# kasirershahartau/tissue_image_processing

Measured on AMD Instinct MI355X. Metric: frames/sec end-to-end (2048^2, z=30), higher is better.
Workload: dtype f32(f16x3)

## Files before the change

include/tissue_hip.h:

```cpp
#ifndef TISSUE_HIP_H
#define TISSUE_HIP_H

#include <stddef.h>
#include <stdint.h>

#ifdef __cplusplus
extern "C" {
#endif

#define TIP_API __attribute__((visibility("default")))

typedef enum {
    TIP_OK = 0,
    TIP_ERR_HIP = -1,
    TIP_ERR_ARG = -2,
    TIP_ERR_NOMEM = -3,
    TIP_ERR_INDEX = -4,
    TIP_ERR_UNSUPPORTED = -5,
    TIP_ERR_OVERFLOW = -6
} tip_status;

TIP_API int tip_init(int device);
TIP_API int tip_shutdown(void);
TIP_API int tip_last_error(char *buf, size_t n);
// ... 52 lines not shown
                                     int ref_ch, int airyscan, int atoh_shift,
                                     const double *t05, const double *t1, const double *t2, const double *t30,
                                     const unsigned long long *hist_dev, double *proj, int64_t *zmap);

TIP_API int tip_bias_relu_affine_f32_dev(float *x, const float *bias, const float *scale, const float *shift, long n, int c,
                                         void *stream);
TIP_API int tip_pointer_device(const void *p);
TIP_API int tip_wait_stream(void *stream);
TIP_API int tip_stream_wait_tip(void *stream);
typedef struct tip_unet_conv_desc {
    const void *in0, *in1;
    int c0, c1, h, w, planes;
    const void *weights;
    int ntaps, dy[9], dx[9];
    int cout;
    const float *bias, *scale, *shift;
    void *out;
    int out_h, out_w, sy, sx, oy, ox;
    void *pool_out;
    const float *head_w, *head_b;
    float *head_out;
    int format;
    float acc_scale;
} tip_unet_conv_desc;
TIP_API int tip_unet_conv_dev(const tip_unet_conv_desc *d, void *stream);
TIP_API int tip_unet_conv_first_dev(const float *in, int h, int w, const float *wgt, const float *bias, const float *scale,
                                    const float *shift, void *out, int planes, int format, void *stream);
TIP_API int tip_unet_pool2_dev(const void *in, int h, int w, int ch, int planes, int format, void *out, void *stream);
TIP_API int tip_unet_head_dev(const void *in, long npix, const float *wgt, const float *bias, float *out, int planes, int format,
                              int logits, void *stream);
TIP_API int tip_unet_prepare_f64_dev(const double *img, int c, int a, int b, long cstride, long sa, long sb, int kind, float *out,
                                     int ap, int bp, void *stream);
TIP_API int tip_unet_tail_dev(const void *p, int dtype, long ld, int y, int x, double thr, int32_t *labels, double *hc,
                              int32_t *flags_host);

TIP_API int tip_draw_cell_types_u8(const uint8_t *types, long n, int must_mask, int lack_mask, const double *pos_rgb,
                                   const double *neg_rgb, double *out3);
TIP_API int tip_draw_tracking_i32(const int32_t *track, long n, const double *cycle18, double *out3);
TIP_API int tip_draw_disks_f64(int y, int x, int n, const double *cy, const double *cx, double radius, const double *rgb, double *out3);
TIP_API int tip_draw_lines_f64(int y, int x, int n, const int32_t *ends, const double *rgb, double *out3);

TIP_API int tip_rankfilter2d(const void *in, void *out, int dtype , int y, int x, int ky, int kx,
                             int footprint_kind, int border_mode, int is_max);
TIP_API int tip_rankfilter2d_dev(const void *in, void *out, int dtype, int y, int x, int ky, int kx,
                                 int footprint_kind, int border_mode, int is_max);
TIP_API int tip_local_threshold_f64_dev(const double *img, double *out, int y, int x, double imgthresh, int block);

TIP_API int tip_label4_i32(const int32_t *in, int32_t bg, int32_t *out, int y, int x, int32_t *n_labels);
// ... 58 lines not shown
```

tissue_image_processing_amd/_unet_hip.py:

```python
import ctypes
import os
import threading

import numpy as np

from . import _lib

_MODES = {
    "f16x3": (2, 1, 3, "7.2e-7"),
    "bf16x3": (2, 0, 3, "1.6e-5"),
    "bf16x6": (3, 0, 6, "9e-8"),
}
_F16_ACT_SCALE = 16.0


class _ConvDesc(ctypes.Structure):
    _fields_ = [("in0", ctypes.c_void_p), ("in1", ctypes.c_void_p), ("c0", ctypes.c_int), ("c1", ctypes.c_int), ("h", ctypes.c_int),
                ("w", ctypes.c_int), ("planes", ctypes.c_int), ("weights", ctypes.c_void_p), ("ntaps", ctypes.c_int),
                ("dy", ctypes.c_int * 9), ("dx", ctypes.c_int * 9), ("cout", ctypes.c_int), ("bias", ctypes.c_void_p),
                ("scale", ctypes.c_void_p), ("shift", ctypes.c_void_p), ("out", ctypes.c_void_p), ("out_h", ctypes.c_int),
                ("out_w", ctypes.c_int), ("sy", ctypes.c_int), ("sx", ctypes.c_int), ("oy", ctypes.c_int), ("ox", ctypes.c_int),
                ("pool_out", ctypes.c_void_p), ("head_w", ctypes.c_void_p), ("head_b", ctypes.c_void_p), ("head_out", ctypes.c_void_p),
                ("format", ctypes.c_int), ("acc_scale", ctypes.c_float)]


def split_pack(taps, planes, fmt=0):
    import torch
    T, cin, cout = taps.shape
    pieces, rest = [], taps.float()
    for _ in range(planes):
        h = rest.to(torch.float16 if fmt else torch.bfloat16)
        pieces.append(h)
        rest = rest - h.float()
    row = torch.arange(32, device=taps.device)
    chan = 16 * ((row >> 2) & 1) + 4 * (row >> 3) + (row & 3)
    pk = torch.stack(pieces, 0).view(planes, T, cin // 16, 16, cout // 32, 32)[..., chan]
    pk = pk.reshape(planes, T, cin // 16, 16, cout // 128, 128)
    return pk.permute(1, 2, 4, 0, 5, 3).contiguous()


def weights(net, mode):
    hw = net._hipw.get(mode)
    if hw is not None:
        return hw
    torch = net.torch
    p = net.p
    planes, fmt = _MODES[mode][:2]
    act = _F16_ACT_SCALE if fmt else 1.0
    hw = {}

    def pack(taps, bias_only):
        if not fmt:
            return split_pack(taps, planes), 1.0
        big = float(taps.abs().max())
        wscale = 2.0 ** (14 - int(np.floor(np.log2(big)))) if big > 0 and np.isfinite(big) else 1.0
        inv = 1.0 / (act * wscale)
        return split_pack(taps * wscale, planes, fmt), (inv * act if bias_only else inv)

    def conv3(name):
        w = p[name + ".w"].float()
        taps = torch.stack([w[:, :, ky, kx].t() for ky in range(3) for kx in range(3)], 0)
        wp, inv = pack(taps, False)
        hw[name] = (wp, [ky - 1 for ky in range(3) for kx in range(3)], [kx - 1 for ky in range(3) for kx in range(3)], inv)

    def conv_t(name):
        w = p[name + ".w"].float()
        per_axis = {0: [(0, 0), (2, -1)], 1: [(1, 0)]}
        for py in (0, 1):
            for px in (0, 1):
                tl = [(ky, dy, kx, dx) for ky, dy in per_axis[py] for kx, dx in per_axis[px]]
                taps = torch.stack([w[:, :, ky, kx] for ky, _, kx, _ in tl], 0)
                wp, inv = pack(taps, True)
                hw["%s.%d%d" % (name, py, px)] = (wp, [t[1] for t in tl], [t[3] for t in tl], inv)

    for blk in ("d0", "d1", "d2", "mid", "u0", "u1", "u2"):
        if blk != "d0":
            conv3(blk + ".c1")
        conv3(blk + ".c2")
    for i in range(3):
        conv_t("u%d.t" % i)
    w0 = p["d0.c1.w"].float()
    hw["first"] = w0.permute(2, 3, 1, 0).reshape(18, 128).contiguous()
    hw["head"] = (p["head.w"].float().reshape(2, 128) / act).contiguous()
    for k in list(p):
        if k.endswith((".b", ".s", ".t")) and not k.endswith(".t.w"):
            v = p[k].float().reshape(-1)
            scaled = k.endswith((".s", ".t", ".t.b"))
            hw["f:" + k] = (v * act if scaled else v).contiguous()
    net._hipw[mode] = hw
    return hw


_FORWARD_GATES = {}
_FORWARD_GATES_LOCK = threading.Lock()


def _forward_gate(device_index):
    with _FORWARD_GATES_LOCK:
        g = _FORWARD_GATES.get(device_index)
        if g is None:
            g = _FORWARD_GATES[device_index] = {"lock": threading.Lock(), "event": None, "stream": None}
        return g


def forward(net, x, mode, logits):
    torch = net.torch
    if os.environ.get("TISSUE_HIP_UNET_SERIAL", "1") == "0":
        return _launch(net, x, mode, logits)
    gate = _forward_gate(x.device.index)
    with gate["lock"]:
        s = torch.cuda.current_stream(x.device)
        if gate["event"] is not None and gate["stream"] != s.cuda_stream:
            s.wait_event(gate["event"])
        out = _launch(net, x, mode, logits)
        ev = torch.cuda.Event()
        ev.record(s)
        gate["event"], gate["stream"] = ev, s.cuda_stream
    return out


def _conv_desc(layer, planes, fmt, src, skip, h, w, bias, scale=None, shift=None, out=None, out_h=None, out_w=None, stride=1, oy=0, ox=0,
               pooled=None, head=None):
    wp, dy, dx, inv = layer
    d = _ConvDesc()
    d.format, d.acc_scale = fmt, inv
    d.in0, d.c0 = src.data_ptr(), src.shape[3]
    d.in1, d.c1 = (skip.data_ptr(), skip.shape[3]) if skip is not None else (None, 0)
    d.h, d.w, d.planes = h, w, planes
    d.weights, d.ntaps, d.cout = wp.data_ptr(), len(dy), wp.shape[2] * 128
    for i in range(len(dy)):
        d.dy[i], d.dx[i] = dy[i], dx[i]
    d.bias = bias.data_ptr()
    d.scale, d.shift = (scale.data_ptr(), shift.data_ptr()) if scale is not None else (None, None)
    if head is not None:
        d.head_w, d.head_b, d.head_out = (t.data_ptr() for t in head)
    d.out = out.data_ptr() if out is not None else None
    d.out_h, d.out_w = (h, w) if out_h is None else (out_h, out_w)
    d.sy, d.sx, d.oy, d.ox = stride, stride, oy, ox
    d.pool_out = pooled.data_ptr() if pooled is not None else None
    return d


def _launch(net, x, mode, logits):
    torch = net.torch
    planes, fmt = _MODES[mode][:2]
    hw = weights(net, mode)
    net.last_mode = mode
    lib = _lib.lib()
    stream = ctypes.c_void_p(torch.cuda.current_stream(x.device).cuda_stream)
    H, W = int(x.shape[2]), int(x.shape[3])
    x = x.to(torch.float32).contiguous()
    D = lambda t: ctypes.c_void_p(t.data_ptr())
    trace = getattr(net, "trace", None)

    def timed(name, flop, fn):
        if trace is None:
            return fn()
        e0, e1 = torch.cuda.Event(enable_timing=True), torch.cuda.Event(enable_timing=True)
        e0.record()
        r = fn()
        e1.record()
        trace.append((name, flop, e0, e1))
        return r

    def buf(h, w, c):
        return torch.empty((planes, h, w, c), dtype=torch.float16 if fmt else torch.bfloat16, device=x.device)

    def launch_conv(name, d):
        timed("%s %dx%d %d+%d->%d x%d taps" % (name, d.h, d.w, d.c0, d.c1, d.cout, d.ntaps), 2.0 * d.h * d.w * d.ntaps * d.cout * (d.c0 + d.c1),
              lambda: _lib.check(lib.tip_unet_conv_dev(ctypes.byref(d), stream)))

    def conv3(name, bn, src, skip, h, w, pooled=None, head=None):
        out = buf(h, w, hw[name][0].shape[2] * 128) if head is None else None
        launch_conv(name, _conv_desc(hw[name], planes, fmt, src, skip, h, w, hw["f:" + name + ".b"], hw["f:" + bn + ".s"], hw["f:" + bn + ".t"],
                                     out=out, pooled=pooled, head=None if head is None else (hw["head"], hw["f:head.b"], head)))
        return out

    def first(h, w):
        out = buf(h, w, 128)
        timed("first %dx%d 2->128" % (h, w), 2.0 * h * w * 18 * 128,
              lambda: _lib.check(lib.tip_unet_conv_first_dev(D(x), h, w, D(hw["first"]), D(hw["f:d0.c1.b"]), D(hw["f:d0.b1.s"]),
                                                             D(hw["f:d0.b1.t"]), D(out), planes, fmt, stream)))
        return out

    def double(blk, src, skip, h, w, pooled=None, head=None):
        a = first(h, w) if src is None else conv3(blk + ".c1", blk + ".b1", src, skip, h, w)
        return conv3(blk + ".c2", blk + ".b2", a, None, h, w, pooled=pooled, head=head)

    def conv_t(name, src, h, w):
        up = buf(2 * h, 2 * w, hw[name + ".00"][0].shape[2] * 128)
        for py in (0, 1):
            for px in (0, 1):
                cls = "%s.%d%d" % (name, py, px)
                launch_conv(cls, _conv_desc(hw[cls], planes, fmt, src, None, h, w, hw["f:" + name + ".b"], out=up, out_h=2 * h, out_w=2 * w,
                                            stride=2, oy=py, ox=px))
        return up

    with torch.no_grad():
        skips, cur, h, w = [], None, H, W
        for i in range(3):
            pooled = buf(h // 2, w // 2, net.filters[i])
            skips.append(double("d%d" % i, cur, None, h, w, pooled=pooled))
            cur, h, w = pooled, h // 2, w // 2
        cur = double("mid", cur, None, h, w)
        for i in range(3):
            up = conv_t("u%d.t" % i, cur, h, w)
            h, w = 2 * h, 2 * w
            probs = None
            if i == 2 and not logits and not os.environ.get("TISSUE_HIP_UNET_SEPARATE_HEAD"):
                probs = torch.empty((1, 2, H, W), dtype=torch.float32, device=x.device)
            cur = double("u%d" % i, up, skips[2 - i], h, w, head=probs)
        if probs is not None:
            return probs
        out = torch.empty((1, 2, H, W), dtype=torch.float32, device=x.device)
        timed("head %dx%d" % (H, W), 2.0 * H * W * 256,
              lambda: _lib.check(lib.tip_unet_head_dev(D(cur), ctypes.c_long(H * W), D(hw["head"]), D(hw["f:head.b"]), D(out), planes, fmt,
                                                       1 if logits else 0, stream)))
    return out
```

tissue_image_processing_amd/csrc/tip_unet.hip:

```cpp
#include "tip_internal.h"
#include "tip_unet_conv.h"
#include <algorithm>
#include <atomic>

namespace tip {

__global__ void __launch_bounds__(256) k_bias_relu_affine_f32(float *__restrict__ x, const float *__restrict__ bias,
                                                              const float *__restrict__ scale, const float *__restrict__ shift,
                                                              long n4, int C)
{
    const long i = (long)blockIdx.x * blockDim.x + threadIdx.x;
    if (i >= n4) return;
    float4 v = reinterpret_cast<float4 *>(x)[i];
    const int c = (int)((i * 4) % C);
    const float4 b = *reinterpret_cast<const float4 *>(bias + c);
    const float4 s = *reinterpret_cast<const float4 *>(scale + c);
    const float4 t = *reinterpret_cast<const float4 *>(shift + c);
    v.x += b.x; v.y += b.y; v.z += b.z; v.w += b.w;
    v.x = v.x > 0.f ? v.x : 0.f; v.y = v.y > 0.f ? v.y : 0.f; v.z = v.z > 0.f ? v.z : 0.f; v.w = v.w > 0.f ? v.w : 0.f;
    v.x = v.x * s.x + t.x; v.y = v.y * s.y + t.y; v.z = v.z * s.z + t.z; v.w = v.w * s.w + t.w;
    reinterpret_cast<float4 *>(x)[i] = v;
}

int rankfilter2d_dev(const void *in, void *out, int dtype, int Y, int X, int ky, int kx, int fp, int border, int is_max);
// ... 341 lines not shown
    split(1.0 / 100.0, r1, g1);
    split(99.0 / 100.0, r99, g99);
    hipLaunchKernelGGL(k_prep_reset, dim3(1), dim3(64), 0, s, st, c, r1, r99);
    const dim3 hgrid((unsigned)cdiv(n, 2048), (unsigned)c);
    for (int shift = 56; shift >= 0; shift -= 8) {
        hipLaunchKernelGGL(k_prep_hist, hgrid, dim3(256), 0, s, img, cstride, n, st, shift);
        hipLaunchKernelGGL(k_prep_pick, dim3(1), dim3(64), 0, s, st, c, shift);
    }
    hipLaunchKernelGGL(k_prep_next, hgrid, dim3(256), 0, s, img, cstride, n, st);
    hipLaunchKernelGGL(k_prep_finish, dim3(1), dim3(64), 0, s, st, c, g1, g99, kind);
    if (ap != a || bp != b) TIP_HIP(hipMemsetAsync(out, 0, (size_t)c * ap * bp * sizeof(float), s));
    const dim3 ngrid((unsigned)cdiv(a, 32), (unsigned)cdiv(b, 32), (unsigned)c);
    if (a_contig)
        hipLaunchKernelGGL(k_prep_normalize<true>, ngrid, dim3(256), 0, s, img, cstride, sa, sb, a, b, (const PrepState *)st, kind == 1 ? 1 : 0, out, ap, bp, ap - a, bp - b);
    else
        hipLaunchKernelGGL(k_prep_normalize<false>, ngrid, dim3(256), 0, s, img, cstride, sa, sb, a, b, (const PrepState *)st, kind == 1 ? 1 : 0, out, ap, bp, ap - a, bp - b);
    return unet_launch_check("unet_prepare");
}

int tip_unet_conv_dev(const tip_unet_conv_desc *d, void *stream)
{
    Ctx &c = ctx();
    if (!c.stream) return TIP_ERR_HIP;
    if (!d || !d->in0 || !d->weights || !d->bias || (!d->out && !d->head_out)) return fail(TIP_ERR_ARG, "tip_unet_conv_dev: null pointer");
    if (d->planes != 2 && d->planes != 3) return fail(TIP_ERR_ARG, "tip_unet_conv_dev: planes must be 2 or 3");
    if (d->format != 0 && d->format != 1) return fail(TIP_ERR_ARG, "tip_unet_conv_dev: format is 0 (bf16 pieces) or 1 (fp16 pieces)");
    if (d->format == 1 && (d->planes != 2 || !(d->acc_scale > 0.f))) return fail(TIP_ERR_ARG, "tip_unet_conv_dev: fp16 pieces come in two planes with a positive acc_scale");
    if (d->h < 8 || d->w < UC_TW || d->h % 8 || d->w % UC_TW)
        return fail(TIP_ERR_UNSUPPORTED, "tip_unet_conv_dev: the grid %dx%d is not a multiple of the 8x%d pixel tile", d->h, d->w, UC_TW);
    if (d->c0 < UC_KC || d->c0 % UC_KC || d->c1 < 0 || d->c1 % UC_KC || (d->c1 > 0 && !d->in1) || d->cout < UC_BN || d->cout % UC_BN)
        return fail(TIP_ERR_UNSUPPORTED, "tip_unet_conv_dev: channels (%d + %d -> %d) must be multiples of %d / %d", d->c0, d->c1, d->cout, UC_KC, UC_BN);
    if (d->ntaps < 1 || d->ntaps > 9 || d->sy < 1 || d->sx < 1 || d->oy < 0 || d->ox < 0 ||
        (d->h - 1) * d->sy + d->oy >= d->out_h || (d->w - 1) * d->sx + d->ox >= d->out_w)
        return fail(TIP_ERR_ARG, "tip_unet_conv_dev: bad taps / output mapping");
    if ((d->scale == nullptr) != (d->shift == nullptr)) return fail(TIP_ERR_ARG, "tip_unet_conv_dev: scale and shift come together");
    if (18L * d->w * (d->c0 > d->c1 ? d->c0 : d->c1) * 2 >= (1L << 32) - 65536)
        return fail(TIP_ERR_UNSUPPORTED, "tip_unet_conv_dev: 18 rows of %d pixels x %d channels exceed the 4 GB a buffer resource addresses",
                    d->w, d->c0 > d->c1 ? d->c0 : d->c1);
    ConvParams p;
    p.in0 = (const uint16_t *)d->in0; p.in1 = (const uint16_t *)(d->c1 > 0 ? d->in1 : d->in0);
    p.c0 = d->c0; p.c1 = d->c1; p.H = d->h; p.W = d->w;
    p.w = (const uint16_t *)d->weights; p.ntaps = d->ntaps;
    for (int t = 0; t < 9; ++t) {
        p.dy[t] = t < d->ntaps ? d->dy[t] : 0; p.dx[t] = t < d->ntaps ? d->dx[t] : 0;
        if (p.dy[t] < -1 || p.dy[t] > 1 || p.dx[t] < -1 || p.dx[t] > 1) return fail(TIP_ERR_ARG, "tip_unet_conv_dev: tap offsets are -1, 0 or 1");
    }
    p.cout = d->cout; p.bias = d->bias; p.scale = d->scale; p.shift = d->shift;
    p.out = (uint16_t *)d->out; p.outH = d->out_h; p.outW = d->out_w; p.sy = d->sy; p.sx = d->sx; p.oy = d->oy; p.ox = d->ox;
    p.pool_out = (uint16_t *)d->pool_out;
    p.acc_scale = d->format == 1 ? d->acc_scale : 1.f;
#ifdef UC_TRACE
    static unsigned long long *trace_dev = nullptr;
    if (!trace_dev) { TIP_HIP(hipMalloc(&trace_dev, 1024)); }
    TIP_HIP(hipMemsetAsync(trace_dev, 0, 1024, (hipStream_t)stream));
    p.trace = trace_dev;
#endif
    p.head_w = d->head_w; p.head_b = d->head_b; p.head_out = d->head_out;
    if (d->head_out && (!d->head_w || !d->head_b || d->cout != UC_BN || !d->scale || d->pool_out || d->sy != 1 || d->sx != 1 || d->oy != 0 || d->ox != 0 ||
                        d->out_h != d->h || d->out_w != d->w))
        return fail(TIP_ERR_ARG, "tip_unet_conv_dev: the fused head needs a 128-channel Conv2D + BatchNorm layer with the plain output mapping");
    if (d->pool_out && (d->sy != 1 || d->sx != 1 || d->oy != 0 || d->ox != 0 || d->out_h != d->h || d->out_w != d->w))
        return fail(TIP_ERR_ARG, "tip_unet_conv_dev: pool_out needs the plain output mapping");
    const int t8 = tuning().unet_tile8;
    const bool want8 = t8 == 1 || (t8 < 0 && d->ntaps == 9 && d->c0 + d->c1 <= 128);
    const int th = (d->planes == 2 && d->h % 16 == 0 && !want8) ? 16 : 8;
    const int dist = (th == 16 && d->ntaps >= 4) ? 4 : 2;
    const int da = (th == 16 && d->ntaps <= 2) ? 2 : 1;
    const int threads = th * 32, hp = UC_HW * (th + 2);
    const int ntiles = (d->h / th) * (d->w / UC_TW), nblks = d->cout / UC_BN;
    p.xcd_map = (tuning().unet_xcd_map && nblks > 1 && ntiles % 8 == 0) ? 1 : 0;
    const dim3 grid = p.xcd_map ? dim3((unsigned)(ntiles * nblks)) : dim3(ntiles, nblks);
    const int a_per = (d->planes * ((hp * 2 + 63) / 64) * 64 + threads - 1) / threads;
    const int spb = (th == 16 && dist == 4 && d->ntaps == 9 && tuning().unet_spb > 1) ? 3 : 1;
    const size_t lds = (size_t)(da + 1) * a_per * threads * 16 + (size_t)(spb > 1 ? 3 * spb : dist + 1) * d->planes * 256 * 16;
    hipStream_t s = (hipStream_t)stream;
    int which;
    if (d->planes == 3) which = 3;
    else if (th == 8) which = 0;
    else if (spb == 3) which = 6;
    else if (dist == 4) which = 2;
    else if (da == 2) which = 4;
    else which = 1;
    static std::atomic<unsigned> attr_done[64];
    const unsigned bit = 1u << (which + (d->format ? 9 : 0));
    const int dev = c.device >= 0 && c.device < 64 ? c.device : 0;
// ... 21 lines not shown
            UC_FLAVOUR(4, k_unet_conv<2, 16, 2, 2, 1, true>)
            UC_FLAVOUR(1, k_unet_conv<2, 16, 2, 1, 1, true>)
            UC_FLAVOUR(0, k_unet_conv<2, 8, 2, 1, 1, true>)
        }
    }
#undef UC_FLAVOUR
#ifdef UC_TRACE
    {
        unsigned long long tr[128];
        TIP_HIP(hipStreamSynchronize(s));
        TIP_HIP(hipMemcpy(tr, trace_dev, sizeof tr, hipMemcpyDeviceToHost));
        for (int k = 0; k < th / 2; ++k) {
            const unsigned long long *t = tr + 16 * k;
            const double n = (double)t[4];
            fprintf(stderr, "UC_TRACE th %d spb %d taps %d cin %d cout %d grid %dx%d wave %d simd %d: per STEP (shader clocks; sums over the loop / steps): copies %.0f, products %.0f (first MFMA out after %.0f), "
                            "vmcnt wait %.0f, barrier %.0f, total %.0f; steps %.0f; whole loop %.0f, prologue %.0f, epilogue %.0f clocks\n",
                    th, spb, d->ntaps, d->c0 + d->c1, d->cout, d->h, d->w, k, (int)((t[7] >> 4) & 3), t[0] / n, t[2] / n, t[1] / n, t[6] / n, (t[3] - t[6]) / n, t[5] / n, n, (double)t[5], (double)t[8], (double)t[9]);
        }
    }
#endif
    return unet_launch_check("unet_conv");
}

int tip_unet_conv_first_dev(const float *in, int h, int w, const float *wgt, const float *bias, const float *scale, const float *shift,
                            void *out, int planes, int format, void *stream)
{
    Ctx &c = ctx();
    if (!c.stream) return TIP_ERR_HIP;
    if (!in || !wgt || !bias || !scale || !shift || !out || h < 1 || w < 1 || w % FIRST_RUN || ((long)h * w) % FIRST_PIX || (planes != 2 && planes != 3) ||
        (format != 0 && !(format == 1 && planes == 2)))
        return fail(TIP_ERR_ARG, "tip_unet_conv_first_dev: bad arguments (w must be a multiple of 32, h * w of 256)");
    const dim3 grid((unsigned)((long)h * w / FIRST_PIX));
    hipStream_t s = (hipStream_t)stream;
    if (format == 1) hipLaunchKernelGGL((k_unet_conv_first<2, true>), grid, dim3(256), 0, s, in, h, w, wgt, bias, scale, shift, (uint16_t *)out);
    else if (planes == 2) hipLaunchKernelGGL(k_unet_conv_first<2>, grid, dim3(256), 0, s, in, h, w, wgt, bias, scale, shift, (uint16_t *)out);
    else hipLaunchKernelGGL(k_unet_conv_first<3>, grid, dim3(256), 0, s, in, h, w, wgt, bias, scale, shift, (uint16_t *)out);
    return unet_launch_check("unet_conv_first");
}

int tip_unet_pool2_dev(const void *in, int h, int w, int ch, int planes, int format, void *out, void *stream)
{
    Ctx &c = ctx();
    if (!c.stream) return TIP_ERR_HIP;
    if (!in || !out || h < 2 || w < 2 || (h & 1) || (w & 1) || ch < 8 || ch % 8 || (planes != 2 && planes != 3) || (format != 0 && !(format == 1 && planes == 2)))
        return fail(TIP_ERR_ARG, "tip_unet_pool2_dev: bad arguments");
    const long n = (long)(h / 2) * (w / 2) * (ch / 8);
// ... 23 lines not shown
```

tissue_image_processing_amd/csrc/tip_unet_conv.h:

```cpp
#pragma once
#include "tip_internal.h"

namespace tip {

typedef __bf16 bf16x8 __attribute__((ext_vector_type(8)));
typedef float f32x16 __attribute__((ext_vector_type(16)));
typedef __bf16 bf16x2 __attribute__((ext_vector_type(2)));
typedef float f32x2 __attribute__((ext_vector_type(2)));
typedef _Float16 f16x8 __attribute__((ext_vector_type(8)));
typedef _Float16 f16x2 __attribute__((ext_vector_type(2)));
constexpr float UC_F16_MAX = 65504.f;

constexpr int UC_TW = 32;
constexpr int UC_BN = 128;
constexpr int UC_KC = 16;
constexpr int UC_HW = UC_TW + 2;

struct ConvParams {
    const uint16_t *in0, *in1;
    int c0, c1;
    int H, W;
    const uint16_t *w;
    int ntaps;
    int dy[9], dx[9];
    int cout;
    const float *bias, *scale, *shift;
    uint16_t *out;
    int outH, outW, sy, sx, oy, ox;
    const float *head_w, *head_b;
    float *head_out;
#ifdef UC_TRACE
    unsigned long long *trace;
#endif
    int xcd_map;
    float acc_scale;
    uint16_t *pool_out;
};

__device__ __forceinline__ unsigned bf16_rne_bits(float v)
{
    const unsigned b = __float_as_uint(v);
    return (b + 0x7fffu + ((b >> 16) & 1u)) >> 16;
}
__device__ __forceinline__ float bf16_bits_to_f32(unsigned h) { return __uint_as_float(h << 16); }
__device__ __forceinline__ float relu_bits(float v) { return __int_as_float(max(__float_as_int(v), 0)); }
__device__ __forceinline__ float fmax_raw(float a, float b)
{
    float r;
    asm("v_max_f32 %0, %1, %2" : "=v"(r) : "v"(a), "v"(b));
    return r;
}
__device__ __forceinline__ float fmax_pair(float v)
{
    float r;
    asm("s_nop 1\n\tv_max_f32_dpp %0, %1, %1 quad_perm:[1,0,3,2] row_mask:0xf bank_mask:0xf" : "=v"(r) : "v"(v));
    return r;
}

typedef __attribute__((address_space(3))) unsigned char lds_byte;
// ... 135 lines not shown
        }
    };
    const int bq = tid & 255;
    const unsigned b_off = (unsigned)(((tid >> 8) * (UC_BN * UC_KC) + (bq >> 1) * UC_KC + (((bq & 1) ^ ((bq >> 4) & 1))) * 8) * 2);
    auto copy_b = [&](int chunk, int tap, int buf) {
        const int soff = ((tap * nchunks + chunk) * nblks + nblk) * (NPL * UC_BN * UC_KC * 2);
        lds_byte *dst = (lds_byte *)(sB + buf * B_BYTES + wave * 64 * 16);
#pragma unroll
        for (int u = 0; u < B_PER; ++u)
            __builtin_amdgcn_raw_ptr_buffer_load_lds(rs_b, dst + u * UC_THREADS * 16, 16, b_off, soff + u * (UC_THREADS / 256) * (UC_BN * UC_KC * 2), 0, 0);
    };

    f32x16 acc[2][4];
#pragma unroll
    for (int m = 0; m < 2; ++m)
#pragma unroll
        for (int n = 0; n < 4; ++n)
#pragma unroll
            for (int i = 0; i < 16; ++i) acc[m][n][i] = 0.f;

    copy_a(0, 0);
    if (DA == 2 && nchunks > 1) copy_a(1, 1);
    for (int s0 = 0; s0 < (PAIR ? 2 * SPB : D) && s0 < nsteps; ++s0) copy_b(s0 / p.ntaps, s0 % p.ntaps, s0);
    uc_wait_barrier<0>();

    const int r = lane & 31, h = lane >> 5;
    const int b_row = r * 2 + (h ^ ((r >> 3) & 1));
    int step = 0;
    int nc = D / p.ntaps, nt = D % p.ntaps;
    int buf0 = 0, buf2 = D;
    uint4 fa[2][NPL], fb[4][NPL];
#ifdef UC_TRACE
    unsigned long long tr_copy = 0, tr_read = 0, tr_mfma = 0, tr_bar = 0, tr_t0 = __builtin_amdgcn_s_memtime();
    const bool tracing = blockIdx.x == gridDim.x / 2 && blockIdx.y == 0;
    unsigned long long tr_wait = 0, t_w = 0;
#define UC_T(var) const unsigned long long var = __builtin_amdgcn_s_memtime()
#define UC_WB t_w = uc_wait_barrier_timed
#else
#define UC_T(var)
#define UC_WB uc_wait_barrier
#endif
#define UC_PRODUCT(PA, PB)                                                                                      \
    _Pragma("unroll") for (int m = 0; m < 2; ++m) _Pragma("unroll") for (int n = 0; n < 4; ++n)                 \
        acc[m][n] = uc_mfma<F16>(fb[n][PB], fa[m][PA], acc[m][n]);
    auto step_products = [&](int chunk, int tap) {
        const unsigned char *abuf = sA + (chunk % (DA + 1)) * A_BYTES;
// ... 111 lines not shown
            buf2 = buf2 + 1 == UC_NBBUF ? 0 : buf2 + 1;
#ifdef UC_TRACE
            UC_T(t_d);
            tr_copy += t_b - t_a; tr_mfma += t_c - t_b; tr_bar += t_d - t_c; tr_wait += t_w - t_c;
#endif
        }
    }
#ifdef UC_TRACE
    if (tracing && p.trace && lane == 0) {
        unsigned long long *tp = p.trace + 16 * wave;
        tp[0] = tr_copy; tp[1] = tr_read; tp[2] = tr_mfma; tp[3] = tr_bar; tp[4] = (unsigned long long)nsteps;
        tp[5] = __builtin_amdgcn_s_memtime() - tr_t0; tp[6] = tr_wait; tp[7] = (unsigned long long)__builtin_amdgcn_s_getreg((31 << 11) | 4);
        tp[8] = tr_t0 - tr_enter;
    }
    const unsigned long long tr_loop_end = __builtin_amdgcn_s_memtime();
#endif
#undef UC_PRODUCT

    constexpr int EP_ROW = 272, EP_BYTES = 32 * EP_ROW;
    static_assert(UC_THREADS / 64 * EP_BYTES <= (DA + 1) * A_BYTES + UC_NBBUF * B_BYTES, "the staging images fit the tile buffers");
    int pxl = lane & 31, hf = lane >> 5;
    asm volatile("" : "+v"(pxl), "+v"(hf));
    unsigned char *ep = smem + wave * EP_BYTES;
    {
        const float *bip = p.bias + nblk * UC_BN + 16 * hf;
        const float *scp = p.scale + nblk * UC_BN + 16 * hf, *shp = p.shift + nblk * UC_BN + 16 * hf;
        const f32x2 inv2 = {p.acc_scale, p.acc_scale};
        auto biased = [&](float a0, float a1, const f32x2 &b) -> f32x2 {
            if constexpr (F16) return __builtin_elementwise_fma(f32x2{a0, a1}, inv2, b);
            else return f32x2{a0, a1} + b;
        };
#pragma unroll
        for (int n = 0; n < 4; ++n) {
#pragma unroll
            for (int q = 0; q < 4; ++q) {
                const float4 b4 = *reinterpret_cast<const float4 *>(bip + n * 32 + q * 4);
                const f32x2 b01 = {b4.x, b4.y}, b23 = {b4.z, b4.w};
                if (p.scale) {
                    const float4 s4 = *reinterpret_cast<const float4 *>(scp + n * 32 + q * 4), t4 = *reinterpret_cast<const float4 *>(shp + n * 32 + q * 4);
                    const f32x2 s01 = {s4.x, s4.y}, s23 = {s4.z, s4.w}, t01 = {t4.x, t4.y}, t23 = {t4.z, t4.w};
#pragma unroll
                    for (int m = 0; m < 2; ++m) {
                        f32x2 v01 = biased(acc[m][n][q * 4 + 0], acc[m][n][q * 4 + 1], b01);
                        f32x2 v23 = biased(acc[m][n][q * 4 + 2], acc[m][n][q * 4 + 3], b23);
                        v01 = __builtin_elementwise_fma(f32x2{relu_bits(v01[0]), relu_bits(v01[1])}, s01, t01);
                        v23 = __builtin_elementwise_fma(f32x2{relu_bits(v23[0]), relu_bits(v23[1])}, s23, t23);
// ... 265 lines not shown
            for (int pl = 0; pl < NPL; ++pl) pc[pl] = *reinterpret_cast<const uint4 *>(in + pl * plane + pix * 128 + part * 16 + g * 8);
#pragma unroll
            for (int e = 0; e < 8; ++e) {
                const float v = split_value<NPL, F16>(pc, e);
                const int c = part * 16 + g * 8 + e;
                z0 = __builtin_fmaf(v, wgt[c], z0);
                z1 = __builtin_fmaf(v, wgt[128 + c], z1);
            }
        }
    }
#pragma unroll
    for (int d = 1; d < 8; d <<= 1) { z0 += __shfl_xor(z0, d, 64); z1 += __shfl_xor(z1, d, 64); }
    if (pix < npix && part == 0) {
        z0 += bias[0]; z1 += bias[1];
        if (logits) { out[pix] = z0; out[npix + pix] = z1; return; }
        const float m = z0 > z1 ? z0 : z1;
        const float e0 = __expf(z0 - m), e1 = __expf(z1 - m);
        const float s = e0 + e1;
        out[pix] = e0 / s;
        out[npix + pix] = e1 / s;
    }
}

}
```

tissue_image_processing_amd/prediction_local.py:

```python
import ctypes
import os

import numpy as np

from . import _lib, _unet_hip
from ._unet_hip import _ConvDesc, _MODES


def find_desired_shape(shape_y, shape_x):
    if shape_y < 1 or shape_x < 1:
        raise UnboundLocalError("find_desired_shape: extents must be >= 1")
    return 1 << (int(shape_y) - 1).bit_length(), 1 << (int(shape_x) - 1).bit_length()


def normalize_channel(image):
    image = np.asarray(image)
    per99 = np.percentile(image, 99)
    per1 = np.percentile(image, 1)
    kind = image.dtype
    clipped = np.where(image > per99, np.asarray(per99).astype(kind), image)
    clipped = np.where(image < per1, np.asarray(per1).astype(kind), clipped)
    if kind == np.float32:
        return (clipped - np.float32(per1)) / np.float32(per99 - per1)
    return (clipped - per1) / (per99 - per1)
# ... 210 lines not shown
            else:
                continue
            self.p[k] = new.to(device=v.device, dtype=v.dtype).view(v.shape)
        self._hipw.clear()

    def _split_pack(self, taps, planes, fmt=0):
        return _unet_hip.split_pack(taps, planes, fmt)

    def _hip_weights(self, mode):
        return _unet_hip.weights(self, mode)

    def hip_path_ok(self, x):
        torch = self.torch
        return (_unet_mode() != "miopen" and x.is_cuda and self.dtype == torch.float32 and x.shape[0] == 1 and x.shape[1] == 2
                and self.filters == _FILTERS and self.bottleneck == 1024
                and x.shape[2] % 64 == 0 and x.shape[3] % 256 == 0 and shares_runtime_with_torch(x))

    def forward(self, x, logits=False):
        torch = self.torch
        F = torch.nn.functional
        if self.hip_path_ok(x):
            return _unet_hip.forward(self, x, _unet_mode(), logits)
        self.last_mode = "miopen"
        with torch.no_grad():
            x = x.to(self.dtype).contiguous(memory_format=torch.channels_last)
            skips = []
            for i in range(3):
                f = self._double(x, "d%d" % i)
                skips.append(f)
                x = F.max_pool2d(f, 2)
            x = self._double(x, "mid")
            for i in range(3):
                n_h, n_w = x.shape[2] * 2, x.shape[3] * 2
                x = F.conv_transpose2d(x, self.p["u%d.t.w" % i], self.p["u%d.t.b" % i], stride=2)[:, :, :n_h, :n_w]
                x = torch.cat([x, skips[2 - i]], dim=1)
                x = self._double(x, "u%d" % i)
            x = F.conv2d(x, self.p["head.w"], self.p["head.b"])
            if logits:
                return x.float()
            return torch.softmax(x.float(), dim=1)

    def flops(self, h, w):
        total = 0
        c, hh, ww = 2, h, w
        for f in self.filters:
            total += 2 * hh * ww * 9 * (c * f + f * f)
# ... 176 lines not shown
```

Baseline: 18.92.

## Compose transposed-conv upsampling with first decoder conv into low-res convolution

Because nothing nonlinear sits between them, each decoder level's transposed convolution is folded algebraically into the following conv's up-path weights. That yields four parity-class convolutions run directly on the low-resolution input, writing raw fp32 partial sums. A new border kernel fixes zero-padding effects at the image edges and per-position bias terms. The skip-path conv then seeds its accumulators from these partials. This removes the upsampled intermediate tensor and the separate transposed-conv pass, at the cost of an fp32 partial buffer round-trip, extra edge-correction launches and changed rounding in the composed weights.

```diff
diff --git a/include/tissue_hip.h b/include/tissue_hip.h
--- a/include/tissue_hip.h
+++ b/include/tissue_hip.h
@@ -98,8 +98,13 @@
     float *head_out;
     int format;
     float acc_scale;
+    float *raw_out;
+    const float *seed;
 } tip_unet_conv_desc;
 TIP_API int tip_unet_conv_dev(const tip_unet_conv_desc *d, void *stream);
+TIP_API int tip_unet_compose_border_dev(const void *x, int planes, int format, int h, int w, int cin, int cout, const float *row_w,
+                                        const float *col_w, const float *corner_w, const float *bias_tab, float *part, float xscale,
+                                        void *stream);
 TIP_API int tip_unet_conv_first_dev(const float *in, int h, int w, const float *wgt, const float *bias, const float *scale,
                                     const float *shift, void *out, int planes, int format, void *stream);
 TIP_API int tip_unet_pool2_dev(const void *in, int h, int w, int ch, int planes, int format, void *out, void *stream);
diff --git a/tissue_image_processing_amd/_unet_hip.py b/tissue_image_processing_amd/_unet_hip.py
--- a/tissue_image_processing_amd/_unet_hip.py
+++ b/tissue_image_processing_amd/_unet_hip.py
@@ -21,7 +21,7 @@
                 ("scale", ctypes.c_void_p), ("shift", ctypes.c_void_p), ("out", ctypes.c_void_p), ("out_h", ctypes.c_int),
                 ("out_w", ctypes.c_int), ("sy", ctypes.c_int), ("sx", ctypes.c_int), ("oy", ctypes.c_int), ("ox", ctypes.c_int),
                 ("pool_out", ctypes.c_void_p), ("head_w", ctypes.c_void_p), ("head_b", ctypes.c_void_p), ("head_out", ctypes.c_void_p),
-                ("format", ctypes.c_int), ("acc_scale", ctypes.c_float)]
+                ("format", ctypes.c_int), ("acc_scale", ctypes.c_float), ("raw_out", ctypes.c_void_p), ("seed", ctypes.c_void_p)]
 
 
 def split_pack(taps, planes, fmt=0):
@@ -39,8 +39,113 @@
     return pk.permute(1, 2, 4, 0, 5, 3).contiguous()
 
 
-def weights(net, mode):
-    hw = net._hipw.get(mode)
+_COMPOSE_LEVELS = (0, 1, 2)
+
+
+def compose_levels():
+    v = os.environ.get("TISSUE_HIP_UNET_COMPOSE", "1").strip()
+    if v == "0":
+        return ()
+    if v in ("", "1"):
+        return _COMPOSE_LEVELS
+    return tuple(sorted({int(t.strip().lstrip("u")) for t in v.split(",") if t.strip()} & {0, 1, 2}))
+
+
+_COMPOSE_AXIS = {0: [(-1, 0, 1), (-1, 1, 2), (0, 1, 0), (0, 2, 1)],
+                 1: [(-1, 0, 2), (0, 0, 0), (0, 1, 1), (0, 2, 2), (1, 2, 0)]}
+_EDGE_TAPS = [(0, -1), (0, 0), (1, -1), (1, 0), (1, 1)]
+
+
+def compose(tw, bt, w1):
+    import torch
+    tw, bt, w1 = tw.double(), bt.double().reshape(-1), w1.double()
+    C = tw.shape[1]
+    wu = w1[:, :C].permute(2, 3, 1, 0)
+    t = tw.permute(2, 3, 0, 1)
+    prod = {}
+
+    def pair(kty, ktx, kwy, kwx):
+        k = (kty, ktx, kwy, kwx)
+        if k not in prod:
+            prod[k] = t[kty, ktx] @ wu[kwy, kwx]
+        return prod[k]
+
+    classes = {}
+    for py in (0, 1):
+        for px in (0, 1):
+            acc = {}
+            for dy, kwy, kty in _COMPOSE_AXIS[py]:
+                for dx, kwx, ktx in _COMPOSE_AXIS[px]:
+                    m = pair(kty, ktx, kwy, kwx)
+                    acc[(dy, dx)] = acc[(dy, dx)] + m if (dy, dx) in acc else m
+            offs = sorted(acc)
+            classes[(py, px)] = (torch.stack([acc[o] for o in offs], 0), [o[0] for o in offs], [o[1] for o in offs])
+    through = torch.einsum("yxco,c->yxo", wu, bt)
+    bias = through.sum((0, 1))
+    bias_tab = torch.zeros((3, 3, bias.numel()), dtype=torch.float64, device=bias.device)
+    for ry in range(3):
+        for rx in range(3):
+            for ky in range(3):
+                for kx in range(3):
+                    if (ry == 0 and ky == 0) or (ry == 2 and ky == 2) or (rx == 0 and kx == 0) or (rx == 2 and kx == 2):
+                        bias_tab[ry, rx] -= through[ky, kx]
+    zero = torch.zeros_like(pair(2, 2, 2, 2))
+    row_w, col_w = [], []
+    for par, off in _EDGE_TAPS:
+        row_w.append(-sum((pair(2, ktx, 2, kwx) for dx, kwx, ktx in _COMPOSE_AXIS[par] if dx == off), zero))
+        col_w.append(-sum((pair(kty, 2, kwy, 2) for dy, kwy, kty in _COMPOSE_AXIS[par] if dy == off), zero))
+    return classes, bias, bias_tab, torch.stack(row_w, 0), torch.stack(col_w, 0), pair(2, 2, 2, 2)
+
+
+def _pack(taps, planes, fmt, bias_only=False):
+    if not fmt:
+        return split_pack(taps, planes), 1.0
+    big = float(taps.abs().max())
+    wscale = 2.0 ** (14 - int(np.floor(np.log2(big)))) if big > 0 and np.isfinite(big) else 1.0
+    inv = 1.0 / (_F16_ACT_SCALE * wscale)
+    return split_pack(taps * wscale, planes, fmt), (inv * _F16_ACT_SCALE if bias_only else inv)
+
+
+def compose_layers(tw, bt, w1, b1, planes, fmt):
+    import torch
+    w1 = w1.float()
+    C = tw.shape[1]
+    classes, bias, bias_tab, row_w, col_w, corner_w = compose(tw, bt, w1)
+    st = {}
+    for (py, px), (taps, dy, dx) in classes.items():
+        wp, inv = _pack(taps.float(), planes, fmt)
+        st["x%d%d" % (py, px)] = (wp, dy, dx, inv)
+    skip = torch.stack([w1[:, C:, ky, kx].t() for ky in range(3) for kx in range(3)], 0)
+    wp, inv = _pack(skip, planes, fmt)
+    st["skip"] = (wp, [ky - 1 for ky in range(3) for kx in range(3)], [kx - 1 for ky in range(3) for kx in range(3)], inv)
+    st["bias"] = (b1.double().reshape(-1) + bias).float().contiguous()
+    st["border"] = tuple(v.float().contiguous() for v in (row_w, col_w, corner_w, bias_tab))
+    return st
+
+
+def composed_up(st, planes, fmt, src, h, w, stream, name="", launch=None):
+    import torch
+    lib = _lib.lib()
+    launch = launch or (lambda name, flop, fn: fn())
+    cin, cout = src.shape[3], st["x00"][0].shape[2] * 128
+    part = torch.empty((2 * h, 2 * w, cout), dtype=torch.float32, device=src.device)
+    for py in (0, 1):
+        for px in (0, 1):
+            layer = st["x%d%d" % (py, px)]
+            d = _conv_desc(layer, planes, fmt, src, None, h, w, None, raw=part, out_h=2 * h, out_w=2 * w, stride=2, oy=py, ox=px)
+            launch("%sx.%d%d %dx%d %d+0->%d x%d taps" % (name, py, px, h, w, cin, cout, d.ntaps), 2.0 * h * w * d.ntaps * cout * cin,
+                   lambda: _lib.check(lib.tip_unet_conv_dev(ctypes.byref(d), stream)))
+    P = lambda t: ctypes.c_void_p(t.data_ptr())
+    row_w, col_w, corner_w, bias_tab = st["border"]
+    launch("%sborder %dx%d %d->%d" % (name, 2 * h, 2 * w, cin, cout), 2.0 * 2.5 * (h + w) * cin * cout,
+           lambda: _lib.check(lib.tip_unet_compose_border_dev(P(src), planes, fmt, h, w, cin, cout, P(row_w), P(col_w), P(corner_w), P(bias_tab),
+                                                              P(part), ctypes.c_float(1.0 / _F16_ACT_SCALE if fmt else 1.0), stream)))
+    return part
+
+
+def weights(net, mode, levels=None):
+    levels = compose_levels() if levels is None else tuple(levels)
+    hw = net._hipw.get((mode, levels))
     if hw is not None:
         return hw
     torch = net.torch
@@ -50,12 +155,7 @@
     hw = {}
 
     def pack(taps, bias_only):
-        if not fmt:
-            return split_pack(taps, planes), 1.0
-        big = float(taps.abs().max())
-        wscale = 2.0 ** (14 - int(np.floor(np.log2(big)))) if big > 0 and np.isfinite(big) else 1.0
-        inv = 1.0 / (act * wscale)
-        return split_pack(taps * wscale, planes, fmt), (inv * act if bias_only else inv)
+        return _pack(taps, planes, fmt, bias_only)
 
     def conv3(name):
         w = p[name + ".w"].float()
@@ -74,11 +174,14 @@
                 hw["%s.%d%d" % (name, py, px)] = (wp, [t[1] for t in tl], [t[3] for t in tl], inv)
 
     for blk in ("d0", "d1", "d2", "mid", "u0", "u1", "u2"):
-        if blk != "d0":
+        if blk != "d0" and not (blk[0] == "u" and int(blk[1]) in levels):
             conv3(blk + ".c1")
         conv3(blk + ".c2")
     for i in range(3):
-        conv_t("u%d.t" % i)
+        if i in levels:
+            hw["u%d.x" % i] = compose_layers(p["u%d.t.w" % i], p["u%d.t.b" % i], p["u%d.c1.w" % i], p["u%d.c1.b" % i], planes, fmt)
+        else:
+            conv_t("u%d.t" % i)
     w0 = p["d0.c1.w"].float()
     hw["first"] = w0.permute(2, 3, 1, 0).reshape(18, 128).contiguous()
     hw["head"] = (p["head.w"].float().reshape(2, 128) / act).contiguous()
@@ -87,7 +190,7 @@
             v = p[k].float().reshape(-1)
             scaled = k.endswith((".s", ".t", ".t.b"))
             hw["f:" + k] = (v * act if scaled else v).contiguous()
-    net._hipw[mode] = hw
+    net._hipw[(mode, levels)] = hw
     return hw
 
 
@@ -120,7 +223,7 @@
 
 
 def _conv_desc(layer, planes, fmt, src, skip, h, w, bias, scale=None, shift=None, out=None, out_h=None, out_w=None, stride=1, oy=0, ox=0,
-               pooled=None, head=None):
+               pooled=None, head=None, raw=None, seed=None):
     wp, dy, dx, inv = layer
     d = _ConvDesc()
     d.format, d.acc_scale = fmt, inv
@@ -130,7 +233,9 @@
     d.weights, d.ntaps, d.cout = wp.data_ptr(), len(dy), wp.shape[2] * 128
     for i in range(len(dy)):
         d.dy[i], d.dx[i] = dy[i], dx[i]
-    d.bias = bias.data_ptr()
+    d.bias = bias.data_ptr() if bias is not None else None
+    d.raw_out = raw.data_ptr() if raw is not None else None
+    d.seed = seed.data_ptr() if seed is not None else None
     d.scale, d.shift = (scale.data_ptr(), shift.data_ptr()) if scale is not None else (None, None)
     if head is not None:
         d.head_w, d.head_b, d.head_out = (t.data_ptr() for t in head)
@@ -144,8 +249,10 @@
 def _launch(net, x, mode, logits):
     torch = net.torch
     planes, fmt = _MODES[mode][:2]
-    hw = weights(net, mode)
+    levels = compose_levels()
+    hw = weights(net, mode, levels)
     net.last_mode = mode
+    net.last_compose = tuple("u%d" % i for i in levels)
     lib = _lib.lib()
     stream = ctypes.c_void_p(torch.cuda.current_stream(x.device).cuda_stream)
     H, W = int(x.shape[2]), int(x.shape[3])
@@ -170,10 +277,12 @@
         timed("%s %dx%d %d+%d->%d x%d taps" % (name, d.h, d.w, d.c0, d.c1, d.cout, d.ntaps), 2.0 * d.h * d.w * d.ntaps * d.cout * (d.c0 + d.c1),
               lambda: _lib.check(lib.tip_unet_conv_dev(ctypes.byref(d), stream)))
 
-    def conv3(name, bn, src, skip, h, w, pooled=None, head=None):
-        out = buf(h, w, hw[name][0].shape[2] * 128) if head is None else None
-        launch_conv(name, _conv_desc(hw[name], planes, fmt, src, skip, h, w, hw["f:" + name + ".b"], hw["f:" + bn + ".s"], hw["f:" + bn + ".t"],
-                                     out=out, pooled=pooled, head=None if head is None else (hw["head"], hw["f:head.b"], head)))
+    def conv3(name, bn, src, skip, h, w, pooled=None, head=None, seed=None):
+        layer, bias = (hw[name], hw["f:" + name + ".b"]) if seed is None else (hw[name[:2] + ".x"]["skip"], hw[name[:2] + ".x"]["bias"])
+        out = buf(h, w, layer[0].shape[2] * 128) if head is None else None
+        launch_conv(name if seed is None else name + ".seeded",
+                    _conv_desc(layer, planes, fmt, src, skip, h, w, bias, hw["f:" + bn + ".s"], hw["f:" + bn + ".t"],
+                               out=out, pooled=pooled, head=None if head is None else (hw["head"], hw["f:head.b"], head), seed=seed))
         return out
 
     def first(h, w):
@@ -183,8 +292,8 @@
                                                              D(hw["f:d0.b1.t"]), D(out), planes, fmt, stream)))
         return out
 
-    def double(blk, src, skip, h, w, pooled=None, head=None):
-        a = first(h, w) if src is None else conv3(blk + ".c1", blk + ".b1", src, skip, h, w)
+    def double(blk, src, skip, h, w, pooled=None, head=None, seed=None):
+        a = first(h, w) if src is None else conv3(blk + ".c1", blk + ".b1", src, skip, h, w, seed=seed)
         return conv3(blk + ".c2", blk + ".b2", a, None, h, w, pooled=pooled, head=head)
 
     def conv_t(name, src, h, w):
@@ -204,12 +313,16 @@
             cur, h, w = pooled, h // 2, w // 2
         cur = double("mid", cur, None, h, w)
         for i in range(3):
-            up = conv_t("u%d.t" % i, cur, h, w)
+            part = composed_up(hw["u%d.x" % i], planes, fmt, cur, h, w, stream, "u%d." % i, timed) if i in levels else None
+            up = conv_t("u%d.t" % i, cur, h, w) if part is None else None
             h, w = 2 * h, 2 * w
             probs = None
             if i == 2 and not logits and not os.environ.get("TISSUE_HIP_UNET_SEPARATE_HEAD"):
                 probs = torch.empty((1, 2, H, W), dtype=torch.float32, device=x.device)
-            cur = double("u%d" % i, up, skips[2 - i], h, w, head=probs)
+            if part is None:
+                cur = double("u%d" % i, up, skips[2 - i], h, w, head=probs)
+            else:
+                cur = double("u%d" % i, skips[2 - i], None, h, w, head=probs, seed=part)
         if probs is not None:
             return probs
         out = torch.empty((1, 2, H, W), dtype=torch.float32, device=x.device)
diff --git a/tissue_image_processing_amd/csrc/tip_unet.hip b/tissue_image_processing_amd/csrc/tip_unet.hip
--- a/tissue_image_processing_amd/csrc/tip_unet.hip
+++ b/tissue_image_processing_amd/csrc/tip_unet.hip
@@ -387,7 +387,7 @@
 {
     Ctx &c = ctx();
     if (!c.stream) return TIP_ERR_HIP;
-    if (!d || !d->in0 || !d->weights || !d->bias || (!d->out && !d->head_out)) return fail(TIP_ERR_ARG, "tip_unet_conv_dev: null pointer");
+    if (!d || !d->in0 || !d->weights || (!d->bias && !d->raw_out) || (!d->out && !d->head_out && !d->raw_out)) return fail(TIP_ERR_ARG, "tip_unet_conv_dev: null pointer");
     if (d->planes != 2 && d->planes != 3) return fail(TIP_ERR_ARG, "tip_unet_conv_dev: planes must be 2 or 3");
     if (d->format != 0 && d->format != 1) return fail(TIP_ERR_ARG, "tip_unet_conv_dev: format is 0 (bf16 pieces) or 1 (fp16 pieces)");
     if (d->format == 1 && (d->planes != 2 || !(d->acc_scale > 0.f))) return fail(TIP_ERR_ARG, "tip_unet_conv_dev: fp16 pieces come in two planes with a positive acc_scale");
@@ -426,6 +426,10 @@
         return fail(TIP_ERR_ARG, "tip_unet_conv_dev: the fused head needs a 128-channel Conv2D + BatchNorm layer with the plain output mapping");
     if (d->pool_out && (d->sy != 1 || d->sx != 1 || d->oy != 0 || d->ox != 0 || d->out_h != d->h || d->out_w != d->w))
         return fail(TIP_ERR_ARG, "tip_unet_conv_dev: pool_out needs the plain output mapping");
+    p.raw_out = d->raw_out; p.seed = d->seed;
+    if (d->raw_out && (d->head_out || d->pool_out)) return fail(TIP_ERR_ARG, "tip_unet_conv_dev: raw output goes without the head and the pooled map");
+    if (d->seed && (d->sy != 1 || d->sx != 1 || d->oy != 0 || d->ox != 0 || d->out_h != d->h || d->out_w != d->w))
+        return fail(TIP_ERR_ARG, "tip_unet_conv_dev: the accumulator seed needs the plain output mapping");
     const int t8 = tuning().unet_tile8;
     const bool want8 = t8 == 1 || (t8 < 0 && d->ntaps == 9 && d->c0 + d->c1 <= 128);
     const int th = (d->planes == 2 && d->h % 16 == 0 && !want8) ? 16 : 8;
@@ -493,6 +497,37 @@
     return unet_launch_check("unet_conv");
 }
 
+int tip_unet_compose_border_dev(const void *x, int planes, int format, int h, int w, int cin, int cout, const float *row_w, const float *col_w,
+                                const float *corner_w, const float *bias_tab, float *part, float xscale, void *stream)
+{
+    Ctx &c = ctx();
+    if (!c.stream) return TIP_ERR_HIP;
+    if (!x || !row_w || !col_w || !corner_w || !bias_tab || !part || (planes != 2 && planes != 3) || (format != 0 && !(format == 1 && planes == 2)) ||
+        h < 1 || w < 1 || cin < 1 || cout < 128 || cout % 128 || !(xscale > 0.f))
+        return fail(TIP_ERR_ARG, "tip_unet_compose_border_dev: bad arguments");
+    hipStream_t s = (hipStream_t)stream;
+    const int H2 = 2 * h, W2 = 2 * w;
+    const long nb = (2L * W2 + 2L * (H2 - 2)) * (cout / 4);
+    hipLaunchKernelGGL(k_unet_compose_edge_bias, dim3((unsigned)cdiv(nb, 256)), dim3(256), 0, s, part, H2, W2, cout, bias_tab);
+    EdgeParams p;
+    p.x = (const uint16_t *)x; p.xplane = (long)h * w * cin; p.planes = planes; p.f16 = format; p.xscale = xscale;
+    p.cin = cin; p.cout = cout; p.part = part;
+    const long wstride = (long)cin * cout;
+    p.L = w; p.x0 = (long)(h - 1) * w * cin; p.xstep = cin; p.tapmask = 0x1f;
+    for (int t = 0; t < 5; ++t) p.wgt[t] = row_w + t * wstride;
+    p.o0 = (long)(H2 - 1) * W2 * cout; p.ostep = cout;
+    hipLaunchKernelGGL(k_unet_compose_edge, dim3((unsigned)cdiv(p.L, EB_J), (unsigned)(cout / EB_CO)), dim3(EB_CO * EB_G), 0, s, p);
+    p.L = h; p.x0 = (long)(w - 1) * cin; p.xstep = (long)w * cin;
+    for (int t = 0; t < 5; ++t) p.wgt[t] = col_w + t * wstride;
+    p.o0 = (long)(W2 - 1) * cout; p.ostep = (long)W2 * cout;
+    hipLaunchKernelGGL(k_unet_compose_edge, dim3((unsigned)cdiv(p.L, EB_J), (unsigned)(cout / EB_CO)), dim3(EB_CO * EB_G), 0, s, p);
+    p.L = 1; p.x0 = ((long)(h - 1) * w + (w - 1)) * cin; p.xstep = cin; p.tapmask = 0x8;
+    for (int t = 0; t < 5; ++t) p.wgt[t] = corner_w;
+    p.o0 = ((long)(H2 - 1) * W2 + (W2 - 2)) * cout; p.ostep = cout;
+    hipLaunchKernelGGL(k_unet_compose_edge, dim3(1, (unsigned)(cout / EB_CO)), dim3(EB_CO * EB_G), 0, s, p);
+    return unet_launch_check("unet_compose_border");
+}
+
 int tip_unet_conv_first_dev(const float *in, int h, int w, const float *wgt, const float *bias, const float *scale, const float *shift,
                             void *out, int planes, int format, void *stream)
 {
diff --git a/tissue_image_processing_amd/csrc/tip_unet_conv.h b/tissue_image_processing_amd/csrc/tip_unet_conv.h
--- a/tissue_image_processing_amd/csrc/tip_unet_conv.h
+++ b/tissue_image_processing_amd/csrc/tip_unet_conv.h
@@ -35,6 +35,8 @@
     int xcd_map;
     float acc_scale;
     uint16_t *pool_out;
+    float *raw_out;
+    const float *seed;
 };
 
 __device__ __forceinline__ unsigned bf16_rne_bits(float v)
@@ -216,6 +218,21 @@
     copy_a(0, 0);
     if (DA == 2 && nchunks > 1) copy_a(1, 1);
     for (int s0 = 0; s0 < (PAIR ? 2 * SPB : D) && s0 < nsteps; ++s0) copy_b(s0 / p.ntaps, s0 % p.ntaps, s0);
+    if (p.seed) {
+        const float up = 1.f / p.acc_scale;
+#pragma unroll
+        for (int m = 0; m < 2; ++m) {
+            const float *sp = p.seed + ((long)(ty0 + wave * 2 + m) * p.W + tx0 + (lane & 31)) * p.cout + nblk * UC_BN + 16 * (lane >> 5);
+#pragma unroll
+            for (int n = 0; n < 4; ++n)
+#pragma unroll
+                for (int q = 0; q < 4; ++q) {
+                    const float4 v = *reinterpret_cast<const float4 *>(sp + n * 32 + q * 4);
+                    acc[m][n][q * 4 + 0] = F16 ? v.x * up : v.x; acc[m][n][q * 4 + 1] = F16 ? v.y * up : v.y;
+                    acc[m][n][q * 4 + 2] = F16 ? v.z * up : v.z; acc[m][n][q * 4 + 3] = F16 ? v.w * up : v.w;
+                }
+        }
+    }
     uc_wait_barrier<0>();
 
     const int r = lane & 31, h = lane >> 5;
@@ -373,6 +390,22 @@
     int pxl = lane & 31, hf = lane >> 5;
     asm volatile("" : "+v"(pxl), "+v"(hf));
     unsigned char *ep = smem + wave * EP_BYTES;
+    if (p.raw_out) {
+#pragma unroll
+        for (int m = 0; m < 2; ++m) {
+            const int y = ty0 + wave * 2 + m;
+            float *op = p.raw_out + ((long)(y * p.sy + p.oy) * p.outW + ((long)(tx0 + pxl) * p.sx + p.ox)) * p.cout + nblk * UC_BN + 16 * hf;
+#pragma unroll
+            for (int n = 0; n < 4; ++n)
+#pragma unroll
+                for (int q = 0; q < 4; ++q) {
+                    float4 v = {acc[m][n][q * 4 + 0], acc[m][n][q * 4 + 1], acc[m][n][q * 4 + 2], acc[m][n][q * 4 + 3]};
+                    if constexpr (F16) { v.x *= p.acc_scale; v.y *= p.acc_scale; v.z *= p.acc_scale; v.w *= p.acc_scale; }
+                    *reinterpret_cast<float4 *>(op + n * 32 + q * 4) = v;
+                }
+        }
+        return;
+    }
     {
         const float *bip = p.bias + nblk * UC_BN + 16 * hf;
         const float *scp = p.scale + nblk * UC_BN + 16 * hf, *shp = p.shift + nblk * UC_BN + 16 * hf;
@@ -684,4 +717,101 @@
     }
 }
 
-}
+constexpr int EB_J = 8, EB_CO = 64, EB_G = 8, EB_CH = 16 * EB_G;
+struct EdgeParams {
+    const uint16_t *x;
+    long xplane;
+    int planes, f16;
+    float xscale;
+    int cin, cout, L;
+    long x0, xstep;
+    const float *wgt[5];
+    int tapmask;
+    float *part;
+    long o0, ostep;
+};
+static __global__ void __launch_bounds__(EB_CO * EB_G) k_unet_compose_edge(const EdgeParams p)
+{
+    __shared__ float xs[EB_J + 2][EB_CH];
+    __shared__ float red[EB_G - 1][2 * EB_J][EB_CO];
+    const int tid = threadIdx.x, col = tid % EB_CO, g = tid / EB_CO;
+    const int j0 = blockIdx.x * EB_J, co = blockIdx.y * EB_CO + col;
+    float a[2][EB_J];
+#pragma unroll
+    for (int jj = 0; jj < EB_J; ++jj) a[0][jj] = a[1][jj] = 0.f;
+    for (int c0 = 0; c0 < p.cin; c0 += EB_CH) {
+        const int nch = min(EB_CH, p.cin - c0);
+        __syncthreads();
+        for (int i = tid; i < (EB_J + 2) * EB_CH; i += EB_CO * EB_G) {
+            const int jj = i / EB_CH, c = i - jj * EB_CH, j = j0 + jj - 1;
+            float v = 0.f;
+            if (c < nch && j >= 0 && j < p.L) {
+                const uint16_t *src = p.x + p.x0 + (long)j * p.xstep + c0 + c;
+                for (int pl = p.planes - 1; pl >= 0; --pl)
+                    v += p.f16 ? uc_piece_value<true>(src[pl * p.xplane]) : uc_piece_value<false>(src[pl * p.xplane]);
+                v *= p.xscale;
+            }
+            xs[jj][c] = v;
+        }
+        __syncthreads();
+        if (g * 16 < nch) {
+#pragma unroll
+            for (int k8 = 0; k8 < 16; k8 += 8) {
+                float w[8][5];
+#pragma unroll
+                for (int u = 0; u < 8; ++u)
+#pragma unroll
+                    for (int t = 0; t < 5; ++t)
+                        w[u][t] = ((p.tapmask >> t) & 1) ? p.wgt[t][(long)(c0 + g * 16 + k8 + u) * p.cout + co] : 0.f;
+#pragma unroll
+                for (int u = 0; u < 8; ++u) {
+                    const int k = g * 16 + k8 + u;
+#pragma unroll
+                    for (int jj = 0; jj < EB_J; ++jj) {
+                        const float xm = xs[jj][k], xc = xs[jj + 1][k], xp = xs[jj + 2][k];
+                        a[0][jj] = __builtin_fmaf(xc, w[u][1], __builtin_fmaf(xm, w[u][0], a[0][jj]));
+                        a[1][jj] = __builtin_fmaf(xp, w[u][4], __builtin_fmaf(xc, w[u][3], __builtin_fmaf(xm, w[u][2], a[1][jj])));
+                    }
+                }
+            }
+        }
+    }
+    if (g > 0) {
+#pragma unroll
+        for (int jj = 0; jj < EB_J; ++jj) { red[g - 1][2 * jj][col] = a[0][jj]; red[g - 1][2 * jj + 1][col] = a[1][jj]; }
+    }
+    __syncthreads();
+    if (g > 0) return;
+#pragma unroll
+    for (int jj = 0; jj < EB_J; ++jj)
+#pragma unroll
+        for (int par = 0; par < 2; ++par) {
+            if (j0 + jj >= p.L || !(p.tapmask & (par ? 0x1c : 0x3))) continue;
+            float v = a[par][jj];
+#pragma unroll
+            for (int q = 0; q < EB_G - 1; ++q) v += red[q][2 * jj + par][col];
+            p.part[p.o0 + (long)(2 * (j0 + jj) + par) * p.ostep + co] += v;
+        }
+}
+
+static __global__ void __launch_bounds__(256) k_unet_compose_edge_bias(float *__restrict__ part, int H2, int W2, int cout, const float *__restrict__ tab)
+{
+    const int c4 = cout / 4;
+    const long i = (long)blockIdx.x * blockDim.x + threadIdx.x;
+    const long npix = 2L * W2 + 2L * (H2 - 2);
+    if (i >= npix * c4) return;
+    const long e = i / c4;
+    const int c = (int)(i - e * c4) * 4;
+    int y, x;
+    if (e < W2) { y = 0; x = (int)e; }
+    else if (e < 2L * W2) { y = H2 - 1; x = (int)(e - W2); }
+    else { const long k = e - 2L * W2; y = 1 + (int)(k >> 1); x = (k & 1) ? W2 - 1 : 0; }
+    const int type = (y == 0 ? 0 : (y == H2 - 1 ? 2 : 1)) * 3 + (x == 0 ? 0 : (x == W2 - 1 ? 2 : 1));
+    float4 *dst = reinterpret_cast<float4 *>(part + ((long)y * W2 + x) * cout + c);
+    const float4 t = *reinterpret_cast<const float4 *>(tab + (long)type * cout + c);
+    float4 v = *dst;
+    v.x += t.x; v.y += t.y; v.z += t.z; v.w += t.w;
+    *dst = v;
+}
+
+}
diff --git a/tissue_image_processing_amd/prediction_local.py b/tissue_image_processing_amd/prediction_local.py
--- a/tissue_image_processing_amd/prediction_local.py
+++ b/tissue_image_processing_amd/prediction_local.py
@@ -256,6 +256,7 @@
         if self.hip_path_ok(x):
             return _unet_hip.forward(self, x, _unet_mode(), logits)
         self.last_mode = "miopen"
+        self.last_compose = ()
         with torch.no_grad():
             x = x.to(self.dtype).contiguous(memory_format=torch.channels_last)
             skips = []
```

Result: faster. 19.80 (median of 6 runs) (+4.6%).
